# jgrss/cultionet

Measured on AMD Instinct MI355X. Metric: train_chips_per_sec, higher is better.
Workload: dtype f32

## Files before the change

cultionet_amd/csrc/cn_conv.hip:

```cpp
#include "cn_common.h"
#include "cn_conv_geom.h"
#include "cn_profile.h"

#include <cstdlib>

#define KC 8

static int cn_reduce_slices(const CnConvGeom& g, hipStream_t stream);

template <int TN, int TM>
__device__ __forceinline__ void cn_igemm_epilogue(const CnConvGeom& g, const f32x16 (&acc)[TN][TM],
                                                  const bool (&pix_ok)[TM], const int (&out_off)[TM], int co_base,
                                                  int half, int grp, int split, int b,
                                                  const float* __restrict__ bias, float* __restrict__ y) {
  const int HWout = g.Hout * g.Wout;
  const bool sliced = g.slice_stride != 0;
  float* yb = sliced ? g.part + (long)(grp * g.splits + split) * g.slice_stride + (long)b * g.Cout * HWout
                     : y + (long)b * g.ybs;
  const bool first = split == 0;
#pragma unroll
  for (int tn = 0; tn < TN; ++tn) {
#pragma unroll
    for (int r = 0; r < 16; ++r) {
      const int co = co_base + tn * 32 + (r & 3) + 8 * (r >> 2) + 4 * half;
      if (co < g.Cout) {
        const float bv = (bias != nullptr && first) ? bias[co] : 0.f;
#pragma unroll
        for (int tm = 0; tm < TM; ++tm) {
          if (pix_ok[tm]) {
            float* dst = yb + (long)co * HWout + out_off[tm];
            const float v = acc[tn][tm][r] + bv;
            if (sliced) {
              *dst = acc[tn][tm][r];
            } else if (g.atomic_out) {
              atomicAdd(dst, v);
            } else if (g.accumulate) {
              *dst += v;
            } else {
              *dst = v;
            }
          }
        }
      }
    }
  }
}

template <int WAVES_N, int TN, int NI_T>
// ... 142 lines not shown
  {                                                                                                        \
    const float* wrow = w_lds + ((t_) * KC + half) * NT + wn * (TN * 32) + l31;                            \
    _Pragma("unroll") for (int tn = 0; tn < TN; ++tn) opa[bf_][tn] = wrow[(2 * (cp_)) * NT + tn * 32];     \
    opb[bf_][0] = in_lds[pix_lds[0] + (2 * (cp_)) * plane + (toff_)];                                      \
    opb[bf_][1] = in_lds[pix_lds[1] + (2 * (cp_)) * plane + (toff_)];                                      \
  }
#define CN_MFMA(bf_)                                                                                       \
  _Pragma("unroll") for (int tn = 0; tn < TN; ++tn) _Pragma("unroll") for (int tm = 0; tm < 2; ++tm)       \
      acc[tn][tm] = __builtin_amdgcn_mfma_f32_32x32x2f32(opa[bf_][tn], opb[bf_][tm], acc[tn][tm], 0, 0, 0);
      int toff_cur = tap_lds[0];
      CN_LOAD_OPS(0, 0, 0, toff_cur);
#pragma unroll 1
      for (int t = 0; t < ntaps; ++t) {
        const int toff_nxt = (t + 1 < ntaps) ? tap_lds[t + 1] : 0;
        CN_LOAD_OPS(1, t, 1, toff_cur);
        CN_MFMA(0);
        CN_LOAD_OPS(0, t, 2, toff_cur);
        CN_MFMA(1);
        CN_LOAD_OPS(1, t, 3, toff_cur);
        CN_MFMA(0);
        if (t + 1 < ntaps) CN_LOAD_OPS(0, t + 1, 0, toff_nxt);
        CN_MFMA(1);
        toff_cur = toff_nxt;
      }
#undef CN_LOAD_OPS
#undef CN_MFMA
    }
#undef CN_PREFETCH
  }

  cn_igemm_epilogue<TN, 2>(g, acc, pix_ok, out_off, n0 + wn * (TN * 32), half, grp, split, b, bias, y);
}

template <int WAVES_N, int TN, int TM, int NV, int RP>
__global__ __launch_bounds__(256, (NV <= 1 ? 2 : 1)) void cn_conv_igemm_vec_kernel(const CnConvGeom g) {
  constexpr int WAVES_M = 4 / WAVES_N;
  constexpr int MT = WAVES_M * TM * 32;
  constexpr int NT = WAVES_N * TN * 32;
  constexpr int WI = (CN_MAX_TAPS * KC * (NT / 4) + 255) / 256;
  constexpr int VS = NV * 1024;
  constexpr bool PADR = RP == 1 || RP == 2;
  constexpr int ODD = RP == 3 ? 1 : 0;
  constexpr int VSS = VS + ODD;
  extern __shared__ __attribute__((aligned(16))) float smem[];
  float* in_lds = smem;
  float* w_lds = smem + g.w_lds_off;
  int* tap_lds = reinterpret_cast<int*>(smem + g.tap_lds_off);

  const int tid = threadIdx.x, lane = tid & 63, wid = tid >> 6;
  const int half = lane >> 5, l31 = lane & 31;
  const int wm = wid / WAVES_N, wn = wid % WAVES_N;

  int bx, by, split;
  if (!cn_xcd_block(g.grid_x, g.grid_y, g.grid_x * g.grid_y * g.splits, bx, by, split)) return;
  int ci_ = 0;
  if (g.interleave) {
    ci_ = bx % g.ncls;
  } else {
#pragma unroll 1
    for (int c = 1; c < g.ncls; ++c)
      if (bx >= g.cls[c].block_begin) ci_ = c;
  }
  const int grp = g.cls[ci_].grp;
  const float* __restrict__ x = g.gx[grp];
  const float* __restrict__ wp = g.gwp[grp];
  const float* __restrict__ bias = g.gbias[grp];
  float* __restrict__ y = g.gy[grp];
  const int Hg = g.cls[ci_].Hg, Wg = g.cls[ci_].Wg, ntaps = g.cls[ci_].ntaps;
  const int vplane = g.cls[ci_].vplane;
  const int min_dy = g.cls[ci_].min_dy, min_dx = g.cls[ci_].min_dx;
  const int oy0 = g.cls[ci_].oy0, ox0 = g.cls[ci_].ox0;
  const int tiles_per_img = g.cls[ci_].tiles_per_img;
  const int tile = g.interleave ? bx / g.ncls : bx - g.cls[ci_].block_begin;
  const int b = tile / tiles_per_img;
  const int m0 = (tile - b * tiles_per_img) * MT;
  const int Win = g.Win;
  const int pitch = PADR ? ((Win + 3) / 4 * 4 + 4) : Win;
  if (tid < ntaps) {
    tap_lds[tid] = PADR ? (g.cls[ci_].dy[tid] - min_dy) * pitch + g.cls[ci_].dx[tid]
                      : (g.cls[ci_].dy[tid] - min_dy) * Win + (g.cls[ci_].dx[tid] - min_dx);
    tap_lds[CN_MAX_TAPS + tid] = g.cls[ci_].wt[tid];
    tap_lds[2 * CN_MAX_TAPS + tid] = g.cls[ci_].dx[tid];
  }
  __syncthreads();
  const int n0 = by * NT;
  const int Mimg = Hg * Wg;
  const int gy0 = m0 / Wg;
  const int HWin = g.Hin * Win;
  const int start = PADR ? (gy0 * g.is + min_dy) * Win : (gy0 * g.is + min_dy) * Win + min_dx;
  const int f0 = (start >> 2) << 2;
  const int sh = start - f0;

  int goff[NV];
  int ldst[NV];
  int ldst2[NV];
#pragma unroll
  for (int i = 0; i < NV; ++i) {
    const int e4 = 4 * (tid + i * 256) - (PADR ? sh : 0);
    const int lim = PADR ? g.cls[ci_].rows * Win : vplane;
    ldst[i] = 0;
    ldst2[i] = 0;
    if (e4 + 3 >= 0 && e4 < lim) {
      const int fq = start + e4 - (PADR ? 0 : sh);
      goff[i] = (fq >= 0 && (ODD ? fq < HWin : fq + 3 < HWin)) ? fq : -1;
      if (RP == 1) {
        const int r = e4 / Win;
        ldst[i] = r * pitch + 4 + (e4 - r * Win);
      } else if (RP == 2) {
        const int ea = e4 < 0 ? e4 + 2 : e4, eb = e4 + 2;
        const int ra = ea / Win, rb = eb / Win;
        ldst[i] = e4 < 0 ? -1 : ra * pitch + 4 + (ea - ra * Win);
        ldst2[i] = eb < lim ? rb * pitch + 4 + (eb - rb * Win) : -1;
      } else {
        ldst[i] = e4;
      }
    } else {
      goff[i] = -2;
    }
  }
  if (PADR) {
    for (int e = tid; e < KC * VS; e += 256) in_lds[e] = 0.f;
  }

  int pix_lds[TM], out_off[TM];
  unsigned colmask[TM];
  bool pix_ok[TM];
#pragma unroll
  for (int tm = 0; tm < TM; ++tm) {
    const int p = m0 + wm * (TM * 32) + tm * 32 + l31;
    pix_ok[tm] = p < Mimg;
    const int pc = pix_ok[tm] ? p : Mimg - 1;
    const int gy = pc / Wg, gx = pc - gy * Wg;
    pix_lds[tm] = PADR ? ((gy - gy0) * g.is) * pitch + 4 + gx * g.is + half * VS
                     : ((gy - gy0) * g.is) * Win + gx * g.is + sh + half * VSS;
    out_off[tm] = (gy * g.os + oy0) * g.Wout + gx * g.os + ox0;
    unsigned m = 0;
    for (int t = 0; t < ntaps; ++t) {
      const int ix = gx * g.is + tap_lds[2 * CN_MAX_TAPS + t];
      if (ix >= 0 && ix < Win) m |= 1u << t;
    }
    colmask[tm] = m;
  }

  f32x16 acc[TN][TM];
#pragma unroll
  for (int tn = 0; tn < TN; ++tn)
#pragma unroll
    for (int tm = 0; tm < TM; ++tm)
#pragma unroll
      for (int r = 0; r < 16; ++r) acc[tn][tm][r] = 0.f;
  const float* xb = x + (long)b * g.xbs;
  const int nw4 = ntaps * KC * (NT / 4);
  const int nchunks = (g.Cin + KC - 1) / KC;
  int ch = split * g.chunks_per_split;
  int ch_end = ch + g.chunks_per_split;
  if (ch_end > nchunks) ch_end = nchunks;

  if (ntaps > 0 && ch < ch_end) {
    f32x4 xin[KC][NV];
    f32x4 win[WI];
    constexpr unsigned CN_OOB = 0x80000000u;
    const __amdgpu_buffer_rsrc_t xrs =
        __builtin_amdgcn_make_buffer_rsrc(const_cast<float*>(xb), 0, 0x7fffffff, 0x00020000);
    const __amdgpu_buffer_rsrc_t wrs =
        __builtin_amdgcn_make_buffer_rsrc(const_cast<float*>(wp), 0, 0x7fffffff, 0x00020000);
    unsigned xo[NV], wo[WI];
#pragma unroll
    for (int i = 0; i < NV; ++i) xo[i] = goff[i] >= 0 ? (unsigned)goff[i] * 4u : CN_OOB;
#pragma unroll
    for (int j = 0; j < WI; ++j) {
      const int f = tid + j * 256;
      wo[j] = CN_OOB;
      if (f < nw4) {
        const int row = f / (NT / 4), c4 = f - row * (NT / 4);
        const int t = row / KC, ci = row - t * KC;
        wo[j] = (unsigned)(((tap_lds[CN_MAX_TAPS + t] * g.Kpad + ci) * g.Npad + n0 + c4 * 4) * 4);
      }
    }
#define CN_PREFETCH_V(c0_)                                                                                 \
  {                                                                                                        \
    const int c0 = (c0_);                                                                                  \
    _Pragma("unroll") for (int ci = 0; ci < KC; ++ci) {                                                    \
      if ((c0 + ci) < g.Cin) {                                                           \
// ... 38 lines not shown
        if (f < nw4) *reinterpret_cast<f32x4*>(w_lds + f * 4) = win[j];
      }
      __syncthreads();
      if (ch + 1 < ch_end) CN_PREFETCH_V((ch + 1) * KC);
#pragma unroll 1
      for (int t = 0; t < ntaps; ++t) {
        const int toff = tap_lds[t];
        const float* wrow = w_lds + (t * KC + half) * NT + wn * (TN * 32) + l31;
        const float* brow[TM];
        int msk[TM];
#pragma unroll
        for (int tm = 0; tm < TM; ++tm) {
          brow[tm] = in_lds + pix_lds[tm] + toff;
          msk[tm] = PADR ? -1 : __builtin_amdgcn_sbfe((int)colmask[tm], t, 1);
        }
#pragma unroll
        for (int cp = 0; cp < KC / 2; ++cp) {
          float a[TN], bb[TM];
#pragma unroll
          for (int tn = 0; tn < TN; ++tn) a[tn] = wrow[(2 * cp) * NT + tn * 32];
#pragma unroll
          for (int tm = 0; tm < TM; ++tm)
            bb[tm] = PADR ? brow[tm][(2 * cp) * VS] : __int_as_float(__float_as_int(brow[tm][(2 * cp) * VSS]) & msk[tm]);
#pragma unroll
          for (int tn = 0; tn < TN; ++tn)
#pragma unroll
            for (int tm = 0; tm < TM; ++tm)
              acc[tn][tm] = __builtin_amdgcn_mfma_f32_32x32x2f32(a[tn], bb[tm], acc[tn][tm], 0, 0, 0);
        }
      }
    }
#undef CN_PREFETCH_V
  }

  cn_igemm_epilogue<TN, TM>(g, acc, pix_ok, out_off, n0 + wn * (TN * 32), half, grp, split, b, bias, y);
}

__global__ void cn_pack_weights_kernel(const float* __restrict__ w, float* __restrict__ wp, int T, int K,
                                       int N, int Kpad, int Npad, long sk, long sn, long st) {
  const long total = (long)T * Kpad * Npad;
  for (long i = blockIdx.x * (long)blockDim.x + threadIdx.x; i < total; i += (long)gridDim.x * blockDim.x) {
    const int n = (int)(i % Npad);
    const long r = i / Npad;
    const int k = (int)(r % Kpad);
    const int t = (int)(r / Kpad);
    wp[i] = (k < K && n < N) ? w[k * sk + n * sn + t * st] : 0.f;
  }
}

struct CnPackDesc {
  const float* w;
  float* wp;
  int T, K, N, Kpad, Npad;
  long sk, sn, st;
};

#define CN_PK_TS 32
#define CN_PK_PITCH (32 * CN_MAX_TAPS + 1)
__global__ __launch_bounds__(256) void cn_pack_weights_batched_kernel(const CnPackDesc* __restrict__ descs) {
  __shared__ float tile[CN_PK_TS * CN_PK_PITCH];
  const CnPackDesc d = descs[blockIdx.y];
  const bool n_slow = d.sn > d.sk;
  const long ss = n_slow ? d.sn : d.sk, sm = n_slow ? d.sk : d.sn;
  const int S = n_slow ? d.N : d.K, M = n_slow ? d.K : d.N;
  const int Spad = n_slow ? d.Npad : d.Kpad, Mpad = n_slow ? d.Kpad : d.Npad;
  if (d.T > CN_MAX_TAPS || d.st != 1 || sm != d.T) {
    const long total = (long)d.T * d.Kpad * d.Npad;
    for (long i = blockIdx.x * (long)blockDim.x + threadIdx.x; i < total; i += (long)gridDim.x * blockDim.x) {
// ... 37 lines not shown
}
extern "C" int cn_conv_kpad(int k_in) { return (k_in + KC - 1) / KC * KC; }

extern "C" int cn_pack_weights_f32(const float* w, float* wp, int T, int K, int N, long sk, long sn, long st,
                                   void* stream) {
  const int Kpad = cn_conv_kpad(K), Npad = cn_conv_npad(N);
  const long total = (long)T * Kpad * Npad;
  const int blocks = (int)((total + 255) / 256 < 2048 ? (total + 255) / 256 : 2048);
  CN_LAUNCH(cn_pack_weights_kernel, dim3(blocks), dim3(256), 0, (hipStream_t)stream, w, wp, T, K, N,
                     Kpad, Npad, sk, sn, st);
  return cn_check_launch();
}

extern "C" int cn_pack_weights_batched_f32(const void* descs, int n, void* stream) {
  if (n <= 0) return CN_OK;
  CN_LAUNCH(cn_pack_weights_batched_kernel, dim3(64, n), dim3(256), 0, (hipStream_t)stream,
                     (const CnPackDesc*)descs);
  return cn_check_launch();
}

template <int WAVES_N, int TN, int TM, int NV, int RP>
static int cn_launch_igemm_v(const float* x, const float* wp, const float* bias, float* y, CnConvGeom& g,
                             int total_tiles, int max_taps, int splits, double flops, hipStream_t stream) {
  constexpr int NT = WAVES_N * TN * 32;
  g.tap_lds_off = g.w_lds_off + (max_taps > 0 ? max_taps : 1) * KC * NT;
  if ((long)g.Cin * g.Hin * g.Win * 4 >= (1L << 31) || (long)(max_taps > 0 ? max_taps : 1) * g.Kpad * g.Npad * 4 >= (1L << 31))
    return CN_ERR_ARG;
  const size_t lds = (size_t)(g.tap_lds_off + 3 * CN_MAX_TAPS + 1) * sizeof(float);
  if (lds > 160 * 1024) return CN_ERR_LDS;
  static bool attr_set = false;
  if (!attr_set) {
    (void)hipFuncSetAttribute((const void*)cn_conv_igemm_vec_kernel<WAVES_N, TN, TM, NV, RP>,
                              hipFuncAttributeMaxDynamicSharedMemorySize, 160 * 1024);
    attr_set = true;
  }
  g.grid_x = total_tiles;
  g.grid_y = (g.Cout + NT - 1) / NT;
  g.splits = splits < 1 ? 1 : splits;
  dim3 grid(cn_xcd_grid((long)g.grid_x * g.grid_y * g.splits));
  cn_prof_name("cn_conv_igemm_vec_kernel<%d, %d, %d, %d, %d>", WAVES_N, TN, TM, NV, RP);
  cn_prof_desc("igemm_vec<%d,%d,%d,%d,%d> G%d B%d %d->%d %dx%d->%dx%d taps%d cls%d is%d os%d grid%dx%dx%d", WAVES_N, TN,
               TM, NV, RP, g.G, g.B, g.Cin, g.Cout, g.Hin, g.Win, g.Hout, g.Wout, max_taps, g.ncls, g.is, g.os,
               total_tiles, (g.Cout + NT - 1) / NT, splits);
  cn_prof_bytes(4.0 * g.G * ((double)g.B * g.Cin * g.Hin * g.Win + (double)g.B * g.Cout * g.Hout * g.Wout / (g.shared_y ? g.G : 1) +
                             (double)(max_taps > 0 ? max_taps : 1) * g.Cin * g.Cout));
  cn_prof_before(stream);
  CN_LAUNCH((cn_conv_igemm_vec_kernel<WAVES_N, TN, TM, NV, RP>), grid, dim3(256), lds, stream, g);
  cn_prof_after(stream, NT == 128 ? 0 : 1, flops);
  const int rrc = cn_reduce_slices(g, stream);
  return rrc != CN_OK ? rrc : cn_check_launch();
}

template <int WAVES_N, int TN, int NI_T>
static int cn_launch_igemm_t(const float* x, const float* wp, const float* bias, float* y, CnConvGeom& g,
                             int total_tiles, int max_taps, int splits, double flops, hipStream_t stream) {
  constexpr int NT = WAVES_N * TN * 32;
  g.tap_lds_off = g.w_lds_off + (max_taps > 0 ? max_taps : 1) * KC * NT;
  if ((long)g.Cin * g.Hin * g.Win * 4 >= (1L << 31) || (long)(max_taps > 0 ? max_taps : 1) * g.Kpad * g.Npad * 4 >= (1L << 31))
    return CN_ERR_ARG;
  const size_t lds = (size_t)(g.tap_lds_off + 3 * CN_MAX_TAPS + 1) * sizeof(float);
  if (lds > 160 * 1024) return CN_ERR_LDS;
  static bool attr_set = false;
  if (!attr_set) {
    (void)hipFuncSetAttribute((const void*)cn_conv_igemm_kernel<WAVES_N, TN, NI_T>,
                              hipFuncAttributeMaxDynamicSharedMemorySize, 160 * 1024);
    attr_set = true;
  }
  g.grid_x = total_tiles;
  g.grid_y = (g.Cout + NT - 1) / NT;
  g.splits = splits < 1 ? 1 : splits;
  dim3 grid(cn_xcd_grid((long)g.grid_x * g.grid_y * g.splits));
  cn_prof_name("cn_conv_igemm_kernel<%d, %d, %d>", WAVES_N, TN, NI_T);
  cn_prof_desc("igemm_dw<%d,%d,%d> G%d B%d %d->%d %dx%d->%dx%d taps%d cls%d is%d os%d grid%dx%dx%d", WAVES_N, TN, NI_T,
               g.G, g.B, g.Cin, g.Cout, g.Hin, g.Win, g.Hout, g.Wout, max_taps, g.ncls, g.is, g.os, total_tiles,
               (g.Cout + NT - 1) / NT, splits);
  cn_prof_bytes(4.0 * g.G * ((double)g.B * g.Cin * g.Hin * g.Win + (double)g.B * g.Cout * g.Hout * g.Wout / (g.shared_y ? g.G : 1) +
                             (double)(max_taps > 0 ? max_taps : 1) * g.Cin * g.Cout));
  cn_prof_before(stream);
  CN_LAUNCH((cn_conv_igemm_kernel<WAVES_N, TN, NI_T>), grid, dim3(256), lds, stream, g);
  cn_prof_after(stream, NT == 128 ? 0 : 1, flops);
// ... 20 lines not shown
      if (t == 0 || k.dy[t] < k.min_dy) k.min_dy = k.dy[t];
      if (t == 0 || k.dx[t] < k.min_dx) k.min_dx = k.dx[t];
      if (t == 0 || k.dy[t] > max_dy) max_dy = k.dy[t];
      if (t == 0 || k.dx[t] > max_dx) max_dx = k.dx[t];
    }
    const int rows = (rows_g - 1) * g.is + (max_dy - k.min_dy) + 1;
    k.pitch = (k.Wg - 1) * g.is + (max_dx - k.min_dx) + 1;
    k.plane = rows * k.pitch;
    k.vplane = (rows * g.Win + (max_dx - k.min_dx) + 4 + 3) / 4 * 4;
    k.rows = rows;
    {
      const int rpitch = (g.Win + 3) / 4 * 4 + 4;
      if ((rows + 1) * rpitch + 4 > p.max_rplane) p.max_rplane = (rows + 1) * rpitch + 4;
    }
    if (-k.min_dx > p.max_absdx) p.max_absdx = -k.min_dx;
    if (max_dx > p.max_absdx) p.max_absdx = max_dx;
    k.tiles_per_img = (Mimg + MT - 1) / MT;
    k.block_begin = p.total_tiles;
    p.total_tiles += g.B * k.tiles_per_img;
    if (k.plane > p.max_plane) p.max_plane = k.plane;
    if (k.vplane > p.max_vplane) p.max_vplane = k.vplane;
    if (k.ntaps > p.max_taps) p.max_taps = k.ntaps;
    p.flops += 2.0 * g.B * Mimg * (double)g.Cout * g.Cin * k.ntaps;
  }
  g.interleave = 0;
  if (g.ncls > 1 && g.want_interleave) {
    bool same = true;
    for (int c = 1; c < g.ncls; ++c) same = same && g.cls[c].tiles_per_img == g.cls[0].tiles_per_img;
    g.interleave = same ? 1 : 0;
  }
  return p;
}

struct CnChoice { int cfg, splits, cps; double cost; };

static double cn_launch_cost(long blocks, int cps, double mt_units, int splits, double out_elems) {
  const double F = 273.0, R = 170.0;
  const double c1 = 36.7 + 0.614 * mt_units, c2 = 30.0 + 1.19 * mt_units;
  const long full = blocks / 512, rem = blocks % 512;
  double c = full * (F + cps * c2);
  if (rem > 0) c += F + cps * (rem > 256 ? c2 : c1);
  if (splits > 1) c += R + out_elems * 4.0 * (2.0 * splits + 1.0) / 8.0e6 * (128.0 / 7.5);
  return c;
}

static thread_local float* g_conv_ws;
static thread_local long g_conv_ws_floats;

static CnChoice cn_choose(const CnConvGeom& g0, const int* mts, int ncfg, int NT, bool allow_split) {
  const int nchunks = (g0.Cin + KC - 1) / KC;
  const int ny = (g0.Cout + NT - 1) / NT;
  const int G = g0.G > 0 ? g0.G : 1;
  const double out_elems = (double)g0.B * g0.Cout * g0.Hout * g0.Wout * (g0.shared_y ? 1 : G);
  CnChoice best = {0, 1, nchunks > 0 ? nchunks : 1, 1e300};
  int forced = 0;
  {
    static const char* dbg = getenv("CN_DBG_SPLITS");
    if (dbg) forced = atoi(dbg) < 1 ? 1 : atoi(dbg);
  }
  long ws_cap = 32;
  if (g_conv_ws != nullptr) {
    const long stride = ((long)g0.B * g0.Cout * g0.Hout * g0.Wout + 3) / 4 * 4;
    ws_cap = g_conv_ws_floats / (stride * G);
  }
  int forced_cfg = -1;
  {
    static const char* dbgc = getenv("CN_DBG_CFG");
    if (dbgc) forced_cfg = atoi(dbgc);
  }
  for (int i = 0; i < ncfg; ++i) {
    if (forced_cfg >= 0 && i != (forced_cfg < ncfg ? forced_cfg : ncfg - 1)) continue;
    CnConvGeom gi = g0;
    const CnPlan p = cn_plan(gi, mts[i]);
    if (p.total_tiles <= 0) continue;
    const long base = (long)p.total_tiles * ny;
    int max_splits = (allow_split && p.max_taps > 0 && nchunks >= 4) ? nchunks / 2 : 1;
    if (max_splits > 32) max_splits = 32;
    if (max_splits > ws_cap) max_splits = ws_cap < 1 ? 1 : (int)ws_cap;
    const double taps = p.total_tiles > 0 ? p.flops / (2.0 * g0.Cout * g0.Cin * (double)mts[i] * p.total_tiles) : 9.0;
    const double chunk_units = (double)mts[i] * NT / 128.0 * (taps < 9.0 ? taps : 9.0) / 9.0;
// ... 54 lines not shown
    if (i + 3 < n && (n & 3) == 0 && (a.ybs & 3) == 0 && (reinterpret_cast<uintptr_t>(yb) & 15) == 0) {
      f32x4 s = *reinterpret_cast<const f32x4*>(p0 + i);
      for (int k = 1; k < a.nsum; ++k) s += *reinterpret_cast<const f32x4*>(p0 + (long)k * a.slice_stride + i);
#pragma unroll
      for (int e = 0; e < 4; ++e) {
        const int c = (int)((i + e) / a.HW);
        for (int j = 0; j < a.nbias; ++j)
          if (a.bias[gi * CN_MAX_GROUPS + j] != nullptr) s[e] += a.bias[gi * CN_MAX_GROUPS + j][c];
      }
      f32x4* d = reinterpret_cast<f32x4*>(yb + i);
      *d = a.accumulate ? *d + s : s;
    } else {
      for (long e = i; e < n && e < i + 4; ++e) {
        float s = p0[e];
        for (int k = 1; k < a.nsum; ++k) s += p0[(long)k * a.slice_stride + e];
        const int c = (int)(e / a.HW);
        for (int j = 0; j < a.nbias; ++j)
          if (a.bias[gi * CN_MAX_GROUPS + j] != nullptr) s += a.bias[gi * CN_MAX_GROUPS + j][c];
        yb[e] = a.accumulate ? yb[e] + s : s;
      }
    }
  }
}

static int cn_finish_split(CnConvGeom& g, const CnPlan& p, int splits, int cps, float* y, hipStream_t stream) {
  (void)y;
  const int nchunks = (g.Cin + KC - 1) / KC;
  g.chunks_per_split = cps > 0 ? cps : (nchunks > 0 ? nchunks : 1);
  if (p.max_taps == 0) g.chunks_per_split = nchunks > 0 ? nchunks : 1;
  g.splits = splits < 1 ? 1 : splits;
  g.atomic_out = g.splits > 1 || (g.G > 1 && g.shared_y);
  g.part = nullptr;
  g.slice_stride = 0;
  if (g.atomic_out) {
    const long stride = ((long)g.B * g.Cout * g.Hout * g.Wout + 3) / 4 * 4;
    if (g_conv_ws != nullptr && stride * g.G * g.splits <= g_conv_ws_floats) {
      g.part = g_conv_ws;
      g.slice_stride = stride;
      return CN_OK;
    }
  }
  if (g.atomic_out && !g.accumulate) {
    const int ny = g.shared_y ? 1 : g.G;
    for (int i = 0; i < ny; ++i)
      if (hipMemsetAsync(g.gy[i], 0, sizeof(float) * (size_t)g.B * g.Cout * g.Hout * g.Wout, stream) != hipSuccess)
        return CN_ERR_LAUNCH;
  }
  return CN_OK;
}

static int cn_reduce_slices(const CnConvGeom& g, hipStream_t stream) {
  if (g.slice_stride == 0) return CN_OK;
  CnReduceArgs a = {};
  a.part = g.part;
  a.slice_stride = g.slice_stride;
  a.ybs = g.ybs; a.B = g.B; a.Cout = g.Cout; a.HW = g.Hout * g.Wout; a.accumulate = g.accumulate;
  if (g.shared_y) {
    a.nsum = g.G * g.splits; a.ngrp = 1; a.y[0] = g.gy[0]; a.nbias = g.G;
    for (int j = 0; j < g.G; ++j) a.bias[j] = g.gbias[j];
  } else {
    a.nsum = g.splits; a.ngrp = g.G; a.nbias = 1;
    for (int i = 0; i < g.G; ++i) { a.y[i] = g.gy[i]; a.bias[i * CN_MAX_GROUPS] = g.gbias[i]; }
  }
  const long n = (long)g.Cout * a.HW;
  long bx = (n + 1023) / 1024;
  if (bx > 1024) bx = 1024;
// ... 263 lines not shown
  if (c64 <= c32x64 && c64 <= c32) { CN_G1_GO(2, 2, 1, 32, 3); }
  if (c32x64 <= c32) { CN_G1_GO(1, 2, 1, 32, 4); }
  CN_G1_GO(1, 1, 1, 32, 4);
#undef CN_G1_GO
}

#include <functional>
static int g_autotune = 0;
static std::unordered_map<uint64_t, CnChoice> g_tuned;
static std::mutex g_tune_mu;

extern "C" int cn_conv_set_autotune(int on) {
  std::lock_guard<std::mutex> lk(g_tune_mu);
  g_autotune = on ? 1 : 0;
  if (!on) g_tuned.clear();
  return CN_OK;
}

static uint64_t cn_tune_key(const CnConvGeom& g, bool vec, int nt, bool allow_split) {
  uint64_t h = 1469598103934665603ull;
  auto mix = [&](long v) { h = (h ^ (uint64_t)v) * 1099511628211ull; };
  mix(g.B); mix(g.Cin); mix(g.Hin); mix(g.Win); mix(g.Cout); mix(g.Hout); mix(g.Wout); mix(g.is); mix(g.os);
  mix(g.ncls); mix(g.G); mix(g.shared_y); mix(vec); mix(nt); mix(allow_split); mix(g_conv_ws != nullptr);
  for (int c = 0; c < g.ncls; ++c) {
    const CnConvClass& k = g.cls[c];
    mix(k.Hg); mix(k.Wg); mix(k.ntaps); mix(k.grp);
    for (int t = 0; t < k.ntaps; ++t) { mix(k.dy[t]); mix(k.dx[t]); }
  }
  return h;
}

static CnChoice cn_autotune(const CnConvGeom& g, const int* mts, int ncfg, int nt, bool allow_split,
                            const CnChoice& model, const std::function<int(const CnChoice&, CnConvGeom&)>& run,
                            hipStream_t stream) {
  static const int split_set[] = {1, 2, 3, 4, 6, 8, 12, 16, 24, 32};
  const int nchunks = (g.Cin + KC - 1) / KC;
  const int ny = (g.Cout + nt - 1) / nt;
  long ws_cap = 32;
  if (g_conv_ws != nullptr) {
    const long stride = ((long)g.B * g.Cout * g.Hout * g.Wout + 3) / 4 * 4;
    ws_cap = g_conv_ws_floats / (stride * (g.G > 0 ? g.G : 1));
  }
  hipEvent_t e0, e1;
  if (hipEventCreate(&e0) != hipSuccess || hipEventCreate(&e1) != hipSuccess) return model;
  CnChoice best = model;
  float best_ms = 1e30f;
  for (int i = 0; i < ncfg; ++i) {
    CnConvGeom gi = g;
    const CnPlan p = cn_plan(gi, mts[i]);
    if (p.total_tiles <= 0) continue;
    int max_splits = (allow_split && p.max_taps > 0 && nchunks >= 4) ? nchunks / 2 : 1;
    if (max_splits > 32) max_splits = 32;
    if (max_splits > ws_cap) max_splits = ws_cap < 1 ? 1 : (int)ws_cap;
    for (int sp : split_set) {
      if (sp > max_splits) break;
      const int cps = (nchunks + sp - 1) / sp;
      const int splits = (nchunks + cps - 1) / cps;
      if (splits != sp) continue;
      if ((long)p.total_tiles * ny * splits > 8192) continue;
      const CnChoice c = {i, splits, cps, 0.0};
      float ms = 0.f;
      bool ok = true;
      for (int rep = 0; rep < 2 && ok; ++rep) {
        CnConvGeom gg = g;
        ok = hipEventRecord(e0, stream) == hipSuccess && run(c, gg) == CN_OK &&
             hipEventRecord(e1, stream) == hipSuccess && hipEventSynchronize(e1) == hipSuccess &&
             hipEventElapsedTime(&ms, e0, e1) == hipSuccess;
      }
      if (ok && ms < best_ms) { best_ms = ms; best = c; }
    }
  }
  (void)hipEventDestroy(e0);
  (void)hipEventDestroy(e1);
  return best;
}

int cn_conv_igemm_launch(CnConvGeom& g, hipStream_t stream) {
  if (g.ncls < 1 || g.ncls > CN_MAX_CLASSES || g.B <= 0 || g.G < 1) return g.B <= 0 ? CN_OK : CN_ERR_ARG;
  g.splits = 1;
  const float* x = g.gx[0]; const float* wp = g.gwp[0]; const float* bias = g.gbias[0]; float* y = g.gy[0];
  g.Kpad = cn_conv_kpad(g.Cin);
  g.Npad = cn_conv_npad(g.Cout);
  const int nt = cn_pick_nt(g.Cout);
  const bool dense_out = g.ybs == (long)g.Cout * g.Hout * g.Wout;
  const bool ws_fits = g_conv_ws != nullptr &&
                       (((long)g.B * g.Cout * g.Hout * g.Wout + 3) / 4 * 4) * g.G * 32 <= g_conv_ws_floats;
  const bool allow_split = dense_out || g.accumulate || ws_fits;
  if (g.G > 1 && g.shared_y && !allow_split) return CN_ERR_ARG;
  const int hw4 = (int)(((long)g.Hin * g.Win) % 4);
  g.odd_planes = (hw4 == 1 && !(g.is > 1 && (long)g.Hin * g.Win > 4096)) ? 1 : 0;
  bool vec = (hw4 == 0 || g.odd_planes) && (g.xbs % 4 == 0);
  if (g.is > 1 && (long)g.Hin * g.Win > 4096) vec = false;
  if ((long)g.Cin * g.Hin * g.Win * 4 >= (1L << 31) || (long)CN_MAX_TAPS * cn_conv_kpad(g.Cin) * g.Npad * 4 >= (1L << 31))
    return CN_ERR_ARG;
  for (int i = 0; i < g.G; ++i) vec = vec && ((reinterpret_cast<uintptr_t>(g.gx[i]) & 15) == 0);
  if (vec) {
    CnConvGeom t = g;
    vec = cn_plan(t, 256).max_vplane <= 4 * 1024;
  }
  static const int mts128[3] = {128, 96, 160};
  static const int mts128d[1] = {128};
  static const int mts256[1] = {256};
  const int* mts = nt == 128 ? (vec ? mts128 : mts128d) : mts256;
  const int ncfg = (nt == 128 && vec) ? 3 : 1;
  auto run = [&](const CnChoice& c, CnConvGeom& gg) -> int {
    if (nt == 128) {
      if (vec) {
        switch (c.cfg) {
          case 1: return cn_launch_vec_cfg<4, 1, 3>(x, wp, bias, y, gg, c.splits, c.cps, stream);
          case 2: return cn_launch_vec_cfg<4, 1, 5>(x, wp, bias, y, gg, c.splits, c.cps, stream);
          default: return cn_launch_vec_cfg<2, 2, 2>(x, wp, bias, y, gg, c.splits, c.cps, stream);
        }
      }
      return cn_launch_dword_cfg<2, 2>(x, wp, bias, y, gg, c.splits, c.cps, stream);
    }
    int rc;
    if (nt == 64) {
      if (vec) return cn_launch_vec_cfg<1, 2, 2>(x, wp, bias, y, gg, c.splits, c.cps, stream);
      rc = cn_launch_dword_cfg<1, 2>(x, wp, bias, y, gg, c.splits, c.cps, stream);
    } else {
      if (vec) return cn_launch_vec_cfg<1, 1, 2>(x, wp, bias, y, gg, c.splits, c.cps, stream);
      rc = cn_launch_dword_cfg<1, 1>(x, wp, bias, y, gg, c.splits, c.cps, stream);
    }
    if (rc == CN_ERR_LDS) {
      CnConvGeom g2 = gg;
      rc = cn_launch_dword_cfg<2, 2>(x, wp, bias, y, g2, c.splits, c.cps, stream);
    }
    return rc;
  };
  CnChoice c = cn_choose(g, mts, ncfg, nt, allow_split);
  if (g_autotune) {
    std::lock_guard<std::mutex> lk(g_tune_mu);
    const uint64_t key = cn_tune_key(g, vec, nt, allow_split);
    auto it = g_tuned.find(key);
    if (it != g_tuned.end()) {
      c = it->second;
    } else if (!g.accumulate && !cn_prof_on()) {
      c = cn_autotune(g, mts, ncfg, nt, allow_split, c, run, stream);
      g_tuned.emplace(key, c);
    }
  }
  return run(c, g);
}

static int cn_set_groups(CnConvGeom& g, int G, const float* const* xs, const float* const* wps,
                         const float* const* biases, float* const* ys) {
  if (G < 1 || G > CN_MAX_GROUPS) return CN_ERR_ARG;
  g.G = G;
  int same = 0;
  for (int i = 0; i < G; ++i) {
    g.gx[i] = xs[i]; g.gwp[i] = wps[i]; g.gbias[i] = biases ? biases[i] : nullptr; g.gy[i] = ys[i];
    if (ys[i] == ys[0]) ++same;
  }
  if (same != G && same != 1) return CN_ERR_ARG;
  for (int i = 1; i < G && same == 1; ++i)
    for (int j = 1; j < i; ++j)
      if (ys[i] == ys[j]) return CN_ERR_ARG;
  g.shared_y = (G > 1 && same == G) ? 1 : 0;
  g.has_bias = 0;
  for (int i = 0; i < G; ++i) g.has_bias |= g.gbias[i] != nullptr;
  return CN_OK;
}

static int cn_gather_conv_g(int G, const float* const* xs, long xbs, const float* const* wps,
                            const float* const* biases, float* const* ys, long ybs, int B, int Cin, int Hin,
                            int Win, int Cout, int Hout, int Wout, int KH, int KW, int stride, const int* pads,
                            const int* dils, int accumulate, hipStream_t stream) {
  if (KH * KW > CN_MAX_TAPS || stride < 1) return CN_ERR_ARG;
  if (Hout <= 0 || Wout <= 0) return CN_OK;
  if (G == 1 && KH == 1 && KW == 1 && stride == 1 && pads[0] == 0 && Hout == Hin && Wout == Win) {
    const int r1 = cn_conv1x1_launch(xs[0], xbs, wps[0], biases ? biases[0] : nullptr, ys[0], ybs, B, Cin, Hin * Win,
// ... 206 lines not shown
```

cultionet_amd/csrc/cn_conv_geom.h:

```cpp
#pragma once
#define CN_MAX_TAPS 9
#define CN_MAX_CLASSES 16
#define CN_MAX_GROUPS 4

struct CnConvClass {
  int Hg, Wg;
  int oy0, ox0;
  int ntaps;
  int dy[CN_MAX_TAPS], dx[CN_MAX_TAPS], wt[CN_MAX_TAPS];
  int min_dy, min_dx;
  int pitch, plane;
  int vplane;
  int rows;
  int tiles_per_img;
  int block_begin;
  int grp;
};

struct CnConvGeom {
  int B, Cin, Hin, Win;
  int Cout, Hout, Wout;
  long xbs, ybs;
  int is, os;
  int Kpad, Npad;
  int w_lds_off;
  int tap_lds_off;
  int chunks_per_split;
  int atomic_out;
  int accumulate, has_bias;
  int G, splits, shared_y;
  int odd_planes;
  int want_interleave;
  int interleave;
  float* part;
  long slice_stride;
  int grid_x, grid_y;
  const float* gx[CN_MAX_GROUPS];
  const float* gwp[CN_MAX_GROUPS];
  const float* gbias[CN_MAX_GROUPS];
  float* gy[CN_MAX_GROUPS];
  int ncls;
  CnConvClass cls[CN_MAX_CLASSES];
};

static inline int cn_conv_out(int in, int k, int stride, int pad, int dil) {
  return (in + 2 * pad - dil * (k - 1) - 1) / stride + 1;
}
static inline int cn_convt_out(int in, int k, int stride, int pad, int out_pad) {
  return (in - 1) * stride - 2 * pad + k + out_pad;
}
static inline int cn_floordiv(int a, int b) { return (a >= 0) ? a / b : -((-a + b - 1) / b); }

static inline int cn_gather_taps(int KH, int KW, int pad, int dil, int* dy, int* dx, int* wt) {
  for (int ky = 0; ky < KH; ++ky)
    for (int kx = 0; kx < KW; ++kx) {
      const int t = ky * KW + kx;
      dy[t] = ky * dil - pad; dx[t] = kx * dil - pad; wt[t] = t;
    }
  return KH * KW;
}

static inline int cn_parity_extent(int out, int p, int stride) { return (out - p + stride - 1) / stride; }

// ... 26 lines not shown
```

Baseline: 391.7.

## Fuse grouped convolutions sharing an output into one summing igemm kernel

Adds a fused variant of the vectorised implicit-GEMM conv kernel. When several groups write to the same output with identical tile geometry, each block loops over all classes and accumulates into one set of registers, then writes once with the summed biases. This avoids atomic or slice-buffer output plus the separate reduction pass. In exchange, per-block work grows, split-K is disabled, and the grid shrinks. A cost model and the autotuner choose between the fused and unfused paths.

```diff
diff --git a/cultionet_amd/csrc/cn_conv.hip b/cultionet_amd/csrc/cn_conv.hip
--- a/cultionet_amd/csrc/cn_conv.hip
+++ b/cultionet_amd/csrc/cn_conv.hip
@@ -8,12 +8,37 @@
 
 static int cn_reduce_slices(const CnConvGeom& g, hipStream_t stream);
 
-template <int TN, int TM>
+template <int TN, int TM, bool FZ = false>
 __device__ __forceinline__ void cn_igemm_epilogue(const CnConvGeom& g, const f32x16 (&acc)[TN][TM],
                                                   const bool (&pix_ok)[TM], const int (&out_off)[TM], int co_base,
                                                   int half, int grp, int split, int b,
                                                   const float* __restrict__ bias, float* __restrict__ y) {
   const int HWout = g.Hout * g.Wout;
+  if (FZ) {
+    float* yb = y + (long)b * g.ybs;
+#pragma unroll
+    for (int tn = 0; tn < TN; ++tn) {
+#pragma unroll
+      for (int r = 0; r < 16; ++r) {
+        const int co = co_base + tn * 32 + (r & 3) + 8 * (r >> 2) + 4 * half;
+        if (co < g.Cout) {
+          float bv = 0.f;
+          if (g.has_bias)
+            for (int j = 0; j < g.G; ++j)
+              if (g.gbias[j] != nullptr) bv += g.gbias[j][co];
+#pragma unroll
+          for (int tm = 0; tm < TM; ++tm) {
+            if (pix_ok[tm]) {
+              float* dst = yb + (long)co * HWout + out_off[tm];
+              const float v = acc[tn][tm][r] + bv;
+              *dst = g.accumulate ? *dst + v : v;
+            }
+          }
+        }
+      }
+    }
+    return;
+  }
   const bool sliced = g.slice_stride != 0;
   float* yb = sliced ? g.part + (long)(grp * g.splits + split) * g.slice_stride + (long)b * g.Cout * HWout
                      : y + (long)b * g.ybs;
@@ -222,8 +247,8 @@
   cn_igemm_epilogue<TN, 2>(g, acc, pix_ok, out_off, n0 + wn * (TN * 32), half, grp, split, b, bias, y);
 }
 
-template <int WAVES_N, int TN, int TM, int NV, int RP>
-__global__ __launch_bounds__(256, (NV <= 1 ? 2 : 1)) void cn_conv_igemm_vec_kernel(const CnConvGeom g) {
+template <int WAVES_N, int TN, int TM, int NV, int RP, bool FZ>
+__device__ __forceinline__ void cn_igemm_vec_body(const CnConvGeom& g) {
   constexpr int WAVES_M = 4 / WAVES_N;
   constexpr int MT = WAVES_M * TM * 32;
   constexpr int NT = WAVES_N * TN * 32;
@@ -243,29 +268,50 @@
 
   int bx, by, split;
   if (!cn_xcd_block(g.grid_x, g.grid_y, g.grid_x * g.grid_y * g.splits, bx, by, split)) return;
-  int ci_ = 0;
-  if (g.interleave) {
-    ci_ = bx % g.ncls;
-  } else {
+  int c_lo = 0;
+  if (!FZ) {
+    if (g.interleave) {
+      c_lo = bx % g.ncls;
+    } else {
 #pragma unroll 1
-    for (int c = 1; c < g.ncls; ++c)
-      if (bx >= g.cls[c].block_begin) ci_ = c;
-  }
-  const int grp = g.cls[ci_].grp;
-  const float* __restrict__ x = g.gx[grp];
-  const float* __restrict__ wp = g.gwp[grp];
-  const float* __restrict__ bias = g.gbias[grp];
-  float* __restrict__ y = g.gy[grp];
-  const int Hg = g.cls[ci_].Hg, Wg = g.cls[ci_].Wg, ntaps = g.cls[ci_].ntaps;
-  const int vplane = g.cls[ci_].vplane;
-  const int min_dy = g.cls[ci_].min_dy, min_dx = g.cls[ci_].min_dx;
-  const int oy0 = g.cls[ci_].oy0, ox0 = g.cls[ci_].ox0;
-  const int tiles_per_img = g.cls[ci_].tiles_per_img;
-  const int tile = g.interleave ? bx / g.ncls : bx - g.cls[ci_].block_begin;
+      for (int c = 1; c < g.ncls; ++c)
+        if (bx >= g.cls[c].block_begin) c_lo = c;
+    }
+  }
+  const int c_hi = FZ ? g.ncls : c_lo + 1;
+  const int Hg = g.cls[c_lo].Hg, Wg = g.cls[c_lo].Wg;
+  const int oy0 = g.cls[c_lo].oy0, ox0 = g.cls[c_lo].ox0;
+  const int tiles_per_img = g.cls[c_lo].tiles_per_img;
+  const int tile = FZ ? bx : (g.interleave ? bx / g.ncls : bx - g.cls[c_lo].block_begin);
   const int b = tile / tiles_per_img;
   const int m0 = (tile - b * tiles_per_img) * MT;
   const int Win = g.Win;
   const int pitch = PADR ? ((Win + 3) / 4 * 4 + 4) : Win;
+  const int n0 = by * NT;
+  const int Mimg = Hg * Wg;
+  const int gy0 = m0 / Wg;
+  const int HWin = g.Hin * Win;
+  if (PADR) {
+    for (int e = tid; e < KC * VS; e += 256) in_lds[e] = 0.f;
+  }
+
+  f32x16 acc[TN][TM];
+#pragma unroll
+  for (int tn = 0; tn < TN; ++tn)
+#pragma unroll
+    for (int tm = 0; tm < TM; ++tm)
+#pragma unroll
+      for (int r = 0; r < 16; ++r) acc[tn][tm][r] = 0.f;
+
+#pragma unroll 1
+  for (int ci_ = c_lo; ci_ < c_hi; ++ci_) {
+  const int grp = g.cls[ci_].grp;
+  const float* __restrict__ x = g.gx[grp];
+  const float* __restrict__ wp = g.gwp[grp];
+  const int ntaps = g.cls[ci_].ntaps;
+  const int vplane = g.cls[ci_].vplane;
+  const int min_dy = g.cls[ci_].min_dy, min_dx = g.cls[ci_].min_dx;
+  if (FZ && ci_ != c_lo) __syncthreads();
   if (tid < ntaps) {
     tap_lds[tid] = PADR ? (g.cls[ci_].dy[tid] - min_dy) * pitch + g.cls[ci_].dx[tid]
                       : (g.cls[ci_].dy[tid] - min_dy) * Win + (g.cls[ci_].dx[tid] - min_dx);
@@ -273,10 +319,6 @@
     tap_lds[2 * CN_MAX_TAPS + tid] = g.cls[ci_].dx[tid];
   }
   __syncthreads();
-  const int n0 = by * NT;
-  const int Mimg = Hg * Wg;
-  const int gy0 = m0 / Wg;
-  const int HWin = g.Hin * Win;
   const int start = PADR ? (gy0 * g.is + min_dy) * Win : (gy0 * g.is + min_dy) * Win + min_dx;
   const int f0 = (start >> 2) << 2;
   const int sh = start - f0;
@@ -308,22 +350,17 @@
       goff[i] = -2;
     }
   }
-  if (PADR) {
-    for (int e = tid; e < KC * VS; e += 256) in_lds[e] = 0.f;
-  }
-
-  int pix_lds[TM], out_off[TM];
+
+  int pix_lds[TM];
   unsigned colmask[TM];
-  bool pix_ok[TM];
 #pragma unroll
   for (int tm = 0; tm < TM; ++tm) {
-    const int p = m0 + wm * (TM * 32) + tm * 32 + l31;
-    pix_ok[tm] = p < Mimg;
-    const int pc = pix_ok[tm] ? p : Mimg - 1;
+    int p = m0 + wm * (TM * 32) + tm * 32 + l31;
+    if (FZ) asm volatile("" : "+v"(p));
+    const int pc = p < Mimg ? p : Mimg - 1;
     const int gy = pc / Wg, gx = pc - gy * Wg;
     pix_lds[tm] = PADR ? ((gy - gy0) * g.is) * pitch + 4 + gx * g.is + half * VS
                      : ((gy - gy0) * g.is) * Win + gx * g.is + sh + half * VSS;
-    out_off[tm] = (gy * g.os + oy0) * g.Wout + gx * g.os + ox0;
     unsigned m = 0;
     for (int t = 0; t < ntaps; ++t) {
       const int ix = gx * g.is + tap_lds[2 * CN_MAX_TAPS + t];
@@ -332,13 +369,6 @@
     colmask[tm] = m;
   }
 
-  f32x16 acc[TN][TM];
-#pragma unroll
-  for (int tn = 0; tn < TN; ++tn)
-#pragma unroll
-    for (int tm = 0; tm < TM; ++tm)
-#pragma unroll
-      for (int r = 0; r < 16; ++r) acc[tn][tm][r] = 0.f;
   const float* xb = x + (long)b * g.xbs;
   const int nw4 = ntaps * KC * (NT / 4);
   const int nchunks = (g.Cin + KC - 1) / KC;
@@ -443,8 +473,31 @@
     }
 #undef CN_PREFETCH_V
   }
-
-  cn_igemm_epilogue<TN, TM>(g, acc, pix_ok, out_off, n0 + wn * (TN * 32), half, grp, split, b, bias, y);
+  }
+
+  int out_off[TM];
+  bool pix_ok[TM];
+#pragma unroll
+  for (int tm = 0; tm < TM; ++tm) {
+    const int p = m0 + wm * (TM * 32) + tm * 32 + l31;
+    pix_ok[tm] = p < Mimg;
+    const int pc = pix_ok[tm] ? p : Mimg - 1;
+    const int gy = pc / Wg, gx = pc - gy * Wg;
+    out_off[tm] = (gy * g.os + oy0) * g.Wout + gx * g.os + ox0;
+  }
+  const int grp = g.cls[c_lo].grp;
+  cn_igemm_epilogue<TN, TM, FZ>(g, acc, pix_ok, out_off, n0 + wn * (TN * 32), half, grp, split, b, g.gbias[grp],
+                                g.gy[grp]);
+}
+
+template <int WAVES_N, int TN, int TM, int NV, int RP>
+__global__ __launch_bounds__(256, (NV <= 1 ? 2 : 1)) void cn_conv_igemm_vec_kernel(const CnConvGeom g) {
+  cn_igemm_vec_body<WAVES_N, TN, TM, NV, RP, false>(g);
+}
+
+template <int WAVES_N, int TN, int TM, int NV, int RP>
+__global__ __launch_bounds__(256, (NV <= 1 ? 2 : 1)) void cn_conv_igemm_vecsum_kernel(const CnConvGeom g) {
+  cn_igemm_vec_body<WAVES_N, TN, TM, NV, RP, true>(g);
 }
 
 __global__ void cn_pack_weights_kernel(const float* __restrict__ w, float* __restrict__ wp, int T, int K,
@@ -548,20 +601,29 @@
   if (!attr_set) {
     (void)hipFuncSetAttribute((const void*)cn_conv_igemm_vec_kernel<WAVES_N, TN, TM, NV, RP>,
                               hipFuncAttributeMaxDynamicSharedMemorySize, 160 * 1024);
+    (void)hipFuncSetAttribute((const void*)cn_conv_igemm_vecsum_kernel<WAVES_N, TN, TM, NV, RP>,
+                              hipFuncAttributeMaxDynamicSharedMemorySize, 160 * 1024);
     attr_set = true;
+  }
+  if (g.fused) {
+    if (g.ncls < 1 || total_tiles % g.ncls != 0 || g.slice_stride != 0 || g.atomic_out) return CN_ERR_ARG;
+    total_tiles /= g.ncls;
+    splits = 1;
   }
   g.grid_x = total_tiles;
   g.grid_y = (g.Cout + NT - 1) / NT;
   g.splits = splits < 1 ? 1 : splits;
   dim3 grid(cn_xcd_grid((long)g.grid_x * g.grid_y * g.splits));
-  cn_prof_name("cn_conv_igemm_vec_kernel<%d, %d, %d, %d, %d>", WAVES_N, TN, TM, NV, RP);
-  cn_prof_desc("igemm_vec<%d,%d,%d,%d,%d> G%d B%d %d->%d %dx%d->%dx%d taps%d cls%d is%d os%d grid%dx%dx%d", WAVES_N, TN,
-               TM, NV, RP, g.G, g.B, g.Cin, g.Cout, g.Hin, g.Win, g.Hout, g.Wout, max_taps, g.ncls, g.is, g.os,
-               total_tiles, (g.Cout + NT - 1) / NT, splits);
+  cn_prof_name(g.fused ? "cn_conv_igemm_vecsum_kernel<%d, %d, %d, %d, %d>" : "cn_conv_igemm_vec_kernel<%d, %d, %d, %d, %d>",
+               WAVES_N, TN, TM, NV, RP);
+  cn_prof_desc("igemm_vec%s<%d,%d,%d,%d,%d> G%d B%d %d->%d %dx%d->%dx%d taps%d cls%d is%d os%d grid%dx%dx%d",
+               g.fused ? "sum" : "", WAVES_N, TN, TM, NV, RP, g.G, g.B, g.Cin, g.Cout, g.Hin, g.Win, g.Hout, g.Wout,
+               max_taps, g.ncls, g.is, g.os, total_tiles, (g.Cout + NT - 1) / NT, splits);
   cn_prof_bytes(4.0 * g.G * ((double)g.B * g.Cin * g.Hin * g.Win + (double)g.B * g.Cout * g.Hout * g.Wout / (g.shared_y ? g.G : 1) +
                              (double)(max_taps > 0 ? max_taps : 1) * g.Cin * g.Cout));
   cn_prof_before(stream);
-  CN_LAUNCH((cn_conv_igemm_vec_kernel<WAVES_N, TN, TM, NV, RP>), grid, dim3(256), lds, stream, g);
+  if (g.fused) CN_LAUNCH((cn_conv_igemm_vecsum_kernel<WAVES_N, TN, TM, NV, RP>), grid, dim3(256), lds, stream, g);
+  else CN_LAUNCH((cn_conv_igemm_vec_kernel<WAVES_N, TN, TM, NV, RP>), grid, dim3(256), lds, stream, g);
   cn_prof_after(stream, NT == 128 ? 0 : 1, flops);
   const int rrc = cn_reduce_slices(g, stream);
   return rrc != CN_OK ? rrc : cn_check_launch();
@@ -648,7 +710,7 @@
   return p;
 }
 
-struct CnChoice { int cfg, splits, cps; double cost; };
+struct CnChoice { int cfg, splits, cps; double cost; int fused; };
 
 static double cn_launch_cost(long blocks, int cps, double mt_units, int splits, double out_elems) {
   const double F = 273.0, R = 170.0;
@@ -662,6 +724,57 @@
 
 static thread_local float* g_conv_ws;
 static thread_local long g_conv_ws_floats;
+
+static bool cn_can_fuse(const CnConvGeom& g) {
+  if (!g.shared_y || g.G < 2 || g.ncls != g.G) return false;
+  unsigned seen = 0;
+  for (int c = 0; c < g.ncls; ++c) {
+    const CnConvClass& k = g.cls[c];
+    if (k.grp < 0 || k.grp >= g.G || (seen >> k.grp & 1u)) return false;
+    seen |= 1u << k.grp;
+    if (k.Hg != g.cls[0].Hg || k.Wg != g.cls[0].Wg || k.oy0 != g.cls[0].oy0 || k.ox0 != g.cls[0].ox0) return false;
+  }
+  return true;
+}
+
+static CnChoice cn_choose_fused(const CnConvGeom& g0, const int* mts, int ncfg, int NT, const CnChoice& unfused,
+                                int forced_splits) {
+  const int nchunks = (g0.Cin + KC - 1) / KC;
+  const int ny = (g0.Cout + NT - 1) / NT;
+  const double out_elems = (double)g0.B * g0.Cout * g0.Hout * g0.Wout;
+  const double slice_units = out_elems * 4.0 / 8.0e6 * (128.0 / 7.5);
+  const int nsl = g0.G * unfused.splits;
+  const long stride = ((long)g0.B * g0.Cout * g0.Hout * g0.Wout + 3) / 4 * 4;
+  double ucost = unfused.cost;
+  if (g_conv_ws != nullptr && stride * nsl <= g_conv_ws_floats) {
+    ucost += (2.0 * nsl + 1.0) * slice_units + 170.0;
+    if (unfused.splits > 1) ucost -= (2.0 * unfused.splits + 1.0) * slice_units + 170.0;
+  } else if (!g0.accumulate) {
+    ucost += slice_units;
+  }
+  CnChoice best = unfused;
+  int forced_cfg = -1;
+  {
+    static const char* dbgc = getenv("CN_DBG_CFG");
+    if (dbgc) forced_cfg = atoi(dbgc);
+  }
+  double bcost = 1e300;
+  for (int i = 0; i < ncfg; ++i) {
+    if (forced_cfg >= 0 && i != (forced_cfg < ncfg ? forced_cfg : ncfg - 1)) continue;
+    CnConvGeom gi = g0;
+    const CnPlan p = cn_plan(gi, mts[i]);
+    if (p.total_tiles <= 0 || p.max_taps <= 0) continue;
+    const double taps = p.flops / (2.0 * g0.Cout * g0.Cin * (double)mts[i] * p.total_tiles);
+    const double chunk_units = (double)mts[i] * NT / 128.0 * (taps < 9.0 ? taps : 9.0) / 9.0;
+    const long fblocks = (long)(p.total_tiles / g0.G) * ny;
+    if (fblocks < 1024 && forced_splits != 1) continue;
+    const double cost = cn_launch_cost(fblocks, g0.G * nchunks, chunk_units, 1, out_elems);
+    if (cost < bcost) { bcost = cost; best = {i, 1, nchunks > 0 ? nchunks : 1, cost, 1}; }
+  }
+  if (bcost >= 1e300) return unfused;
+  if (forced_splits) return forced_splits == 1 ? best : unfused;
+  return bcost < ucost ? best : unfused;
+}
 
 static CnChoice cn_choose(const CnConvGeom& g0, const int* mts, int ncfg, int NT, bool allow_split) {
   const int nchunks = (g0.Cin + KC - 1) / KC;
@@ -782,6 +895,12 @@
   g.atomic_out = g.splits > 1 || (g.G > 1 && g.shared_y);
   g.part = nullptr;
   g.slice_stride = 0;
+  if (g.fused) {
+    g.splits = 1;
+    g.chunks_per_split = nchunks > 0 ? nchunks : 1;
+    g.atomic_out = 0;
+    return CN_OK;
+  }
   if (g.atomic_out) {
     const long stride = ((long)g.B * g.Cout * g.Hout * g.Wout + 3) / 4 * 4;
     if (g_conv_ws != nullptr && stride * g.G * g.splits <= g_conv_ws_floats) {
@@ -1111,7 +1230,7 @@
 
 static CnChoice cn_autotune(const CnConvGeom& g, const int* mts, int ncfg, int nt, bool allow_split,
                             const CnChoice& model, const std::function<int(const CnChoice&, CnConvGeom&)>& run,
-                            hipStream_t stream) {
+                            hipStream_t stream, bool can_fuse) {
   static const int split_set[] = {1, 2, 3, 4, 6, 8, 12, 16, 24, 32};
   const int nchunks = (g.Cin + KC - 1) / KC;
   const int ny = (g.Cout + nt - 1) / nt;
@@ -1124,6 +1243,17 @@
   if (hipEventCreate(&e0) != hipSuccess || hipEventCreate(&e1) != hipSuccess) return model;
   CnChoice best = model;
   float best_ms = 1e30f;
+  auto time_one = [&](const CnChoice& c) {
+    float ms = 0.f;
+    bool ok = true;
+    for (int rep = 0; rep < 2 && ok; ++rep) {
+      CnConvGeom gg = g;
+      ok = hipEventRecord(e0, stream) == hipSuccess && run(c, gg) == CN_OK &&
+           hipEventRecord(e1, stream) == hipSuccess && hipEventSynchronize(e1) == hipSuccess &&
+           hipEventElapsedTime(&ms, e0, e1) == hipSuccess;
+    }
+    if (ok && ms < best_ms) { best_ms = ms; best = c; }
+  };
   for (int i = 0; i < ncfg; ++i) {
     CnConvGeom gi = g;
     const CnPlan p = cn_plan(gi, mts[i]);
@@ -1137,17 +1267,9 @@
       const int splits = (nchunks + cps - 1) / cps;
       if (splits != sp) continue;
       if ((long)p.total_tiles * ny * splits > 8192) continue;
-      const CnChoice c = {i, splits, cps, 0.0};
-      float ms = 0.f;
-      bool ok = true;
-      for (int rep = 0; rep < 2 && ok; ++rep) {
-        CnConvGeom gg = g;
-        ok = hipEventRecord(e0, stream) == hipSuccess && run(c, gg) == CN_OK &&
-             hipEventRecord(e1, stream) == hipSuccess && hipEventSynchronize(e1) == hipSuccess &&
-             hipEventElapsedTime(&ms, e0, e1) == hipSuccess;
-      }
-      if (ok && ms < best_ms) { best_ms = ms; best = c; }
-    }
+      time_one({i, splits, cps, 0.0, 0});
+    }
+    if (can_fuse && p.max_taps > 0) time_one({i, 1, nchunks > 0 ? nchunks : 1, 0.0, 1});
   }
   (void)hipEventDestroy(e0);
   (void)hipEventDestroy(e1);
@@ -1183,6 +1305,7 @@
   const int* mts = nt == 128 ? (vec ? mts128 : mts128d) : mts256;
   const int ncfg = (nt == 128 && vec) ? 3 : 1;
   auto run = [&](const CnChoice& c, CnConvGeom& gg) -> int {
+    gg.fused = (c.fused && vec) ? 1 : 0;
     if (nt == 128) {
       if (vec) {
         switch (c.cfg) {
@@ -1208,6 +1331,11 @@
     return rc;
   };
   CnChoice c = cn_choose(g, mts, ncfg, nt, allow_split);
+  const bool can_fuse = vec && cn_can_fuse(g);
+  if (can_fuse) {
+    static const char* dbg = getenv("CN_DBG_SPLITS");
+    c = cn_choose_fused(g, mts, ncfg, nt, c, dbg ? (atoi(dbg) < 1 ? 1 : atoi(dbg)) : 0);
+  }
   if (g_autotune) {
     std::lock_guard<std::mutex> lk(g_tune_mu);
     const uint64_t key = cn_tune_key(g, vec, nt, allow_split);
@@ -1215,7 +1343,7 @@
     if (it != g_tuned.end()) {
       c = it->second;
     } else if (!g.accumulate && !cn_prof_on()) {
-      c = cn_autotune(g, mts, ncfg, nt, allow_split, c, run, stream);
+      c = cn_autotune(g, mts, ncfg, nt, allow_split, c, run, stream, can_fuse);
       g_tuned.emplace(key, c);
     }
   }
diff --git a/cultionet_amd/csrc/cn_conv_geom.h b/cultionet_amd/csrc/cn_conv_geom.h
--- a/cultionet_amd/csrc/cn_conv_geom.h
+++ b/cultionet_amd/csrc/cn_conv_geom.h
@@ -29,6 +29,7 @@
   int atomic_out;
   int accumulate, has_bias;
   int G, splits, shared_y;
+  int fused;
   int odd_planes;
   int want_interleave;
   int interleave;
```

Measured after the change: 380.3. -2.9%, worse.
